# versmc/cmpt-eigenex

Measured on AMD Instinct MI355X. Metric: lanczos_krylov_iterations_per_second, higher is better.
Workload: dtype f64

## Files before the change

### cmpt-eigenex_amd/csrc/kernels.hip

```cpp
#include "kernels.hpp"

#include <algorithm>
#include <cstdlib>
#include <type_traits>

namespace eigenex {

namespace {

__device__ __forceinline__ double wave_sum(double x) {
#pragma unroll
  for (int off = 32; off > 0; off >>= 1) x += __shfl_down(x, off, 64);
  return x;
}

__device__ __forceinline__ double block_sum(double x, double* lds4) {
  x = wave_sum(x);
  const int lane = threadIdx.x & 63, wave = threadIdx.x >> 6;
  __syncthreads();
  if (lane == 0) lds4[wave] = x;
  __syncthreads();
  return (lds4[0] + lds4[1]) + (lds4[2] + lds4[3]);
}

// ... 243 lines not shown
  for (int i = threadIdx.x; i < (DUAL ? 8 : 4) * nacc; i += kBlock) lds[i] = 0.0;
  __syncthreads();
  double a = 0.0;
  if (fin.partials) {
    a = inline_fin_sum(fin, lds4);
    if (blockIdx.x == 0 && threadIdx.x == 0) {
      fin.out[0] = a;
      fin_alpha_apply(fin.ctrl, a, fin.series, fin.mode == kFinishAlphaFirst);
    }
  } else if (tt.uk) {
    a = *tt.a;
  }
  const double b = (tt.uk && tt.ukm1) ? *tt.b : 0.0;
  double* wave_acc = lds + wave * nacc;
  double* wave_acc2 = lds + (4 + wave) * nacc;
  for (int64_t tile = blockIdx.x; tile < ntiles; tile += gridDim.x) {
    const int64_t base = tile * kTileRows + 2 * threadIdx.x;
    if ((tile + 1) * kTileRows <= n)
      dots_tile<true, CPLX, RED4, DUAL>(src, tt, a, b, src2, cs, ncols, base, n, wave_acc, wave_acc2);
    else
      dots_tile<false, CPLX, RED4, DUAL>(src, tt, a, b, src2, cs, ncols, base, n, wave_acc, wave_acc2);
  }
  __syncthreads();
  for (int c = threadIdx.x; c < nacc; c += kBlock) {
    partials[(int64_t)c * pstride + blockIdx.x] = (lds[c] + lds[nacc + c]) + (lds[2 * nacc + c] + lds[3 * nacc + c]);
    if (DUAL) {
      const double* l2 = lds + 4 * nacc;
      partials2[(int64_t)c * pstride + blockIdx.x] = (l2[c] + l2[nacc + c]) + (l2[2 * nacc + c] + l2[3 * nacc + c]);
    }
  }
}

template <bool CPLX>
__device__ __forceinline__ void axmy8(double2 (&w)[4], const double* __restrict__ h, int ci, const double2 (&x)[4]) {
  if (!CPLX) {
    const double hr = h[ci];
#pragma unroll
    for (int i = 0; i < 4; ++i) {
      w[i].x = fma(-hr, x[i].x, w[i].x);
      w[i].y = fma(-hr, x[i].y, w[i].y);
    }
  } else {
    const double hr = h[2 * ci], hi = h[2 * ci + 1];
#pragma unroll
    for (int i = 0; i < 4; ++i) {
      w[i].x = fma(hi, x[i].y, fma(-hr, x[i].x, w[i].x));
      w[i].y = fma(-hi, x[i].x, fma(-hr, x[i].y, w[i].y));
    }
  }
}

template <bool FULL, bool CPLX>
__device__ __forceinline__ double update_tile(const double* src, double* dst,
                                              const ThreeTerm& tt, double a, double b, const ColumnSet& cs, int ncols,
                                              int ntail, const double* __restrict__ h, int64_t base, int64_t n) {
  double2 w[4], uk[4], ukm1[4];
  load_w0<FULL>(w, src, tt, a, b, base, n, &uk, &ukm1);
  const int nv = cs.count - ntail;
  auto from_memory = [&](int lo, int hi) {
    int ci = lo;
    for (; ci + 4 <= hi; ci += 4) {
      double2 x0[4], x1[4], x2[4], x3[4];
      load_col<FULL>(x0, column_ptr(cs, ci + 0), base, n);
      load_col<FULL>(x1, column_ptr(cs, ci + 1), base, n);
      load_col<FULL>(x2, column_ptr(cs, ci + 2), base, n);
      load_col<FULL>(x3, column_ptr(cs, ci + 3), base, n);
      axmy8<CPLX>(w, h, ci + 0, x0);
      axmy8<CPLX>(w, h, ci + 1, x1);
      axmy8<CPLX>(w, h, ci + 2, x2);
      axmy8<CPLX>(w, h, ci + 3, x3);
    }
    for (; ci < hi; ++ci) {
      double2 x0[4];
      load_col<FULL>(x0, column_ptr(cs, ci), base, n);
      axmy8<CPLX>(w, h, ci, x0);
    }
  };
  from_memory(0, nv);
  if (ntail == 2) axmy8<CPLX>(w, h, cs.count - 2, ukm1);
  if (ntail >= 1) axmy8<CPLX>(w, h, cs.count - 1, uk);
  from_memory(cs.count, ncols);
  double nrm = 0.0;
#pragma unroll
  for (int i = 0; i < 4; ++i) {
    const int64_t row = base + i * (2 * kBlock);
    if (FULL || row < n) {
      nt_st2(dst + row, w[i]);
      nrm = fma(w[i].x, w[i].x, nrm);
      nrm = fma(w[i].y, w[i].y, nrm);
    }
  }
  return nrm;
}

template <bool CPLX, bool RED>
__global__ __launch_bounds__(kBlock) void k_update(const double* src, double* dst, ThreeTerm tt, ColumnSet cs,
                                                   const double* __restrict__ h, int64_t n, int64_t ntiles,
                                                   double* __restrict__ partials, const Ctrl* __restrict__ ctrl, InlineReduce red) {
  extern __shared__ double h_lds[];
  __shared__ double lds4[4];
  if (ctrl->stopped) return;
  const int ncols = cs.count + cs.nq;
  const double a = tt.uk ? *tt.a : 0.0;
  const double b = (tt.uk && tt.ukm1) ? *tt.b : 0.0;
  const int ntail = tail_columns(tt, cs);
  if (RED) {
    for (int c = 0; c < red.ncoef; ++c) {
      const double* p = red.partials + (int64_t)c * red.pstride;
      double sc = 0.0;
      for (int bb = threadIdx.x; bb < red.nblocks; bb += kBlock) sc += p[bb];
      sc = block_sum(sc, lds4);
      if (threadIdx.x == 0) h_lds[c] = sc;
    }
    __syncthreads();
    if (blockIdx.x == 0)
      for (int c = threadIdx.x; c < red.ncoef; c += kBlock) red.out[c] = h_lds[c];
  }
  const double* hh = RED ? h_lds : h;
  double nrm = 0.0;
  for (int64_t tile = blockIdx.x; tile < ntiles; tile += gridDim.x) {
    const int64_t base = tile * kTileRows + 2 * threadIdx.x;
    if ((tile + 1) * kTileRows <= n)
      nrm += update_tile<true, CPLX>(src, dst, tt, a, b, cs, ncols, ntail, hh, base, n);
    else
      nrm += update_tile<false, CPLX>(src, dst, tt, a, b, cs, ncols, ntail, hh, base, n);
  }
  nrm = block_sum(nrm, lds4);
  if (threadIdx.x == 0) partials[blockIdx.x] = nrm;
}

__global__ __launch_bounds__(kBlock) void k_reduce(const double* __restrict__ partials, int pstride, int nblocks,
                                                   double* __restrict__ out, const Ctrl* __restrict__ ctrl) {
  __shared__ double lds4[4];
  if (ctrl->stopped) return;
  const double* p = partials + (int64_t)blockIdx.x * pstride;
  double s = 0.0;
  for (int b = threadIdx.x; b < nblocks; b += kBlock) s += p[b];
  s = block_sum(s, lds4);
  if (threadIdx.x == 0) out[blockIdx.x] = s;
}

__device__ __forceinline__ void lag_apply8(double2 (&u)[4], double2 (&w)[4], double cj, double fj, bool with_w, const double2 (&x)[4]) {
#pragma unroll
  for (int i = 0; i < 4; ++i) {
    u[i].x = fma(-cj, x[i].x, u[i].x);
    u[i].y = fma(-cj, x[i].y, u[i].y);
    if (with_w) {
      w[i].x = fma(-fj, x[i].x, w[i].x);
      w[i].y = fma(-fj, x[i].y, w[i].y);
    }
  }
}

template <bool FULL, bool CORRECT>
__device__ __forceinline__ double sweep_tile(const SweepStep& st, double scale, double a, double b, const double* cl, const double* fl,
                                             double* wave_acc, int64_t base, int64_t n) {
  const int lane = threadIdx.x & 63;
  const int k = st.k;
  const double* ukm1 = st.V + (int64_t)(k - 1) * st.ldv;
  double* ukcol = const_cast<double*>(st.V) + (int64_t)k * st.ldv;
  double2 w0[4], w[4], u[4], um[4];
#pragma unroll
  for (int i = 0; i < 4; ++i) {
    const int64_t row = base + i * (2 * kBlock);
    u[i] = w0[i] = w[i] = um[i] = make_double2(0.0, 0.0);
    if (FULL || row < n) {
      const double2 t = ld2(st.w + row);
      u[i] = make_double2(t.x * scale, t.y * scale);
      if (!CORRECT) {
        double2 s = ld2(st.v + row);
        s.x = fma(-a, u[i].x, s.x);
        s.y = fma(-a, u[i].y, s.y);
        if (k > 0) {
          um[i] = ld2(ukm1 + row);
          s.x = fma(-b, um[i].x, s.x);
          s.y = fma(-b, um[i].y, s.y);
        }
        w0[i] = w[i] = s;
      }
    }
  }
  const int nv = CORRECT ? k : (k > 0 ? k - 1 : 0);
  int ci = 0;
  for (; ci + 4 <= nv; ci += 4) {
    double2 x0[4], x1[4], x2[4], x3[4];
    load_col<FULL>(x0, st.V + (int64_t)(ci + 0) * st.ldv, base, n);
    load_col<FULL>(x1, st.V + (int64_t)(ci + 1) * st.ldv, base, n);
    load_col<FULL>(x2, st.V + (int64_t)(ci + 2) * st.ldv, base, n);
    load_col<FULL>(x3, st.V + (int64_t)(ci + 3) * st.ldv, base, n);
    if (!CORRECT) {
      double r0, r1, r2, r3, im;
      dotc8<false>(w0, x0, r0, im);
      dotc8<false>(w0, x1, r1, im);
      dotc8<false>(w0, x2, r2, im);
      dotc8<false>(w0, x3, r3, im);
      const double kr = wave_sum4(r0, r1, r2, r3, lane);
      if ((lane & 15) == 0) wave_acc[ci + (lane >> 4)] += kr;
    }
    lag_apply8(u, w, cl[ci + 0], CORRECT ? 0.0 : fl[ci + 0], !CORRECT, x0);
    lag_apply8(u, w, cl[ci + 1], CORRECT ? 0.0 : fl[ci + 1], !CORRECT, x1);
    lag_apply8(u, w, cl[ci + 2], CORRECT ? 0.0 : fl[ci + 2], !CORRECT, x2);
    lag_apply8(u, w, cl[ci + 3], CORRECT ? 0.0 : fl[ci + 3], !CORRECT, x3);
  }
  for (; ci < nv; ++ci) {
    double2 x0[4];
    load_col<FULL>(x0, st.V + (int64_t)ci * st.ldv, base, n);
    if (!CORRECT) {
      double r0, im;
      dotc8<false>(w0, x0, r0, im);
      r0 = wave_sum(r0);
      if (lane == 0) wave_acc[ci] += r0;
    }
    lag_apply8(u, w, cl[ci], CORRECT ? 0.0 : fl[ci], !CORRECT, x0);
  }
  double nrm = 0.0;
  if (!CORRECT) {
    double r0, r1 = 0.0, im;
    if (k > 0) {
      dotc8<false>(w0, um, r1, im);
      lag_apply8(u, w, cl[k - 1], fl[k - 1], true, um);
    }
    dotc8<false>(w0, u, r0, im);
    const double fk = fl[k];
#pragma unroll
    for (int i = 0; i < 4; ++i) {
      w[i].x = fma(-fk, u[i].x, w[i].x);
      w[i].y = fma(-fk, u[i].y, w[i].y);
    }
    r0 = wave_sum(r0);
    if (k > 0) r1 = wave_sum(r1);
    if (lane == 0) {
      wave_acc[k] += r0;
      if (k > 0) wave_acc[k - 1] += r1;
    }
  }
#pragma unroll
  for (int i = 0; i < 4; ++i) {
    const int64_t row = base + i * (2 * kBlock);
    if (FULL || row < n) {
      nt_st2(ukcol + row, u[i]);
      if (!CORRECT) {
        nt_st2(st.w + row, w[i]);
        nrm = fma(w[i].x, w[i].x, nrm);
        nrm = fma(w[i].y, w[i].y, nrm);
      }
    }
  }
  return nrm;
}

template <bool CORRECT>
__global__ __launch_bounds__(kBlock) void k_sweep(SweepStep st, InlineFin fin, int64_t n, int64_t ntiles, double* __restrict__ dpartials,
                                                  int pstride, double* __restrict__ npartials, const Ctrl* ctrl) {
  extern __shared__ double lds[];
  __shared__ double lds4[4];
  if (ctrl->stopped) return;
  const int k = st.k, nacc = k + 1;
  double* cl = lds + 4 * nacc;
  double* fl = cl + nacc;
  for (int i = threadIdx.x; i < 4 * nacc; i += kBlock) lds[i] = 0.0;
  for (int i = threadIdx.x; i < nacc; i += kBlock) cl[i] = i < k ? st.lag[kLagC + i] : 0.0;
  const double a = fin.partials ? inline_fin_sum(fin, lds4) : *st.a_raw;
  __syncthreads();
  const double da = lag_alpha_correction(k, st.beta, cl);
  if (!CORRECT) {
    for (int i = threadIdx.x; i < nacc; i += kBlock) {
      const double fi = lag_f_entry(i, k, st.alpha, st.beta, cl, a, da);
      fl[i] = fi;
      if (blockIdx.x == 0) st.lag[st.f_off + i] = fi;
    }
  }
  if (blockIdx.x == 0 && threadIdx.x == 0) {
    st.lag[0] = a;
    if (fin.partials) {
      fin.out[0] = a;
      fin_alpha_apply(fin.ctrl, a - da, fin.series, fin.mode == kFinishAlphaFirst);
    } else if (k > 0) {
      st.alpha[k] = a - da;
    }
  }
  __syncthreads();
  const double scale = *st.scale;
  const double b = k > 0 ? st.beta[k - 1] : 0.0;
  double* wave_acc = lds + (threadIdx.x >> 6) * nacc;
  double nrm = 0.0;
  for (int64_t tile = blockIdx.x; tile < ntiles; tile += gridDim.x) {
    const int64_t base = tile * kTileRows + 2 * threadIdx.x;
    if ((tile + 1) * kTileRows <= n)
      nrm += sweep_tile<true, CORRECT>(st, scale, a, b, cl, fl, wave_acc, base, n);
    else
      nrm += sweep_tile<false, CORRECT>(st, scale, a, b, cl, fl, wave_acc, base, n);
  }
  if (CORRECT) return;
  __syncthreads();
  for (int c = threadIdx.x; c < nacc; c += kBlock)
    dpartials[(int64_t)c * pstride + blockIdx.x] = (lds[c] + lds[nacc + c]) + (lds[2 * nacc + c] + lds[3 * nacc + c]);
  nrm = block_sum(nrm, lds4);
  if (threadIdx.x == 0) npartials[blockIdx.x] = nrm;
}

constexpr int kLagWaves = 16;
__global__ __launch_bounds__(64 * kLagWaves) void k_lag_terms(int k, const double* __restrict__ dpartials, int pstride, int nblocks,
                                                              const double* __restrict__ npartials, double* lag, int f_off, double threshold,
                                                              Ctrl* ctrl, Ctrl* repair) {
  __shared__ double lds4[4];
  __shared__ double wmax[kLagWaves];
  if (ctrl->stopped) {
    if (threadIdx.x == 0) repair->stopped = 1;
    return;
  }
  const int lane = threadIdx.x & 63, wave = threadIdx.x >> 6, nwaves = blockDim.x >> 6;
  if (wave < kBlock / 64) {
    double s = 0.0;
    for (int b = threadIdx.x; b < nblocks; b += kBlock) s += npartials[b];
    s = wave_sum(s);
    if (lane == 0) lds4[wave] = s;
  }
  __syncthreads();
  const double beta = sqrt((lds4[0] + lds4[1]) + (lds4[2] + lds4[3]));
  double m = 0.0;
  for (int c = wave; c <= k; c += nwaves) {
    const double* p = dpartials + (int64_t)c * pstride;
    double d = 0.0;
    for (int b = lane; b < nblocks; b += 64) d += p[b];
    d = wave_sum(d);
    if (lane == 0) {
      const double cc = lag_next_coefficient(d, lag[f_off + c], beta, threshold);
      lag[kLagC + c] = cc;
      m = fmax(m, fabs(cc));
    }
  }
  if (lane == 0) wmax[wave] = m;
  __syncthreads();
  double mx = 0.0;
  for (int w = 0; w < nwaves; ++w) mx = fmax(mx, wmax[w]);
  const bool armed = mx > kLagGuard;
  if (armed)
    for (int c = threadIdx.x; c <= k; c += blockDim.x) lag[kLagC + c] = 0.0;
  if (threadIdx.x == 0) {
    repair->stopped = armed ? 0 : 1;
    if (armed) ctrl->repairs++;
  }
}

__global__ void k_close_scalars(int k, const double* a_raw, double* alpha, const double* __restrict__ beta, double* lag, const Ctrl* __restrict__ ctrl) {
  if (ctrl->stopped) return;
  const double a = *a_raw;
  const double da = lag_alpha_correction(k, beta, lag + kLagC);
  lag[0] = a;
  if (k > 0) alpha[k] = a - da;
}

__device__ __forceinline__ void cheb_store(const ChebStep& ch, int64_t r, double a, double x) {
  const double tp = ch.first ? x : ch.t_prev[r];
  const double acc = ch.first ? 0.0 : ch.acc[r];
  double acc_new;
  const double t = cheb_row_nofma(a, tp, acc, ch, &acc_new);
  __builtin_nontemporal_store(t, &ch.t_next[r]);
  __builtin_nontemporal_store(acc_new, &ch.acc[r]);
}

template <bool FULL>
__device__ __forceinline__ void cheb_tile(const double* __restrict__ y, const ChebStep& ch, int64_t base, int64_t n) {
  double2 a[4], tp[4], ac[4];
#pragma unroll
  for (int i = 0; i < 4; ++i) {
    const int64_t row = base + i * (2 * kBlock);
    a[i] = tp[i] = ac[i] = make_double2(0.0, 0.0);
    if (FULL || row < n) {
      a[i] = nt_ld_d2(y + row);
      tp[i] = ld2(ch.t_prev + row);
      if (!ch.first) ac[i] = ld2(ch.acc + row);
    }
  }
#pragma unroll
  for (int i = 0; i < 4; ++i) {
    const int64_t row = base + i * (2 * kBlock);
    if (FULL || row < n) {
      double2 t, an;
      t.x = cheb_row_nofma(a[i].x, tp[i].x, ac[i].x, ch, &an.x);
      t.y = cheb_row_nofma(a[i].y, tp[i].y, ac[i].y, ch, &an.y);
      nt_st2(ch.t_next + row, t);
      nt_st2(ch.acc + row, an);
    }
  }
}

__global__ __launch_bounds__(kBlock) void k_cheb_combine(const double* __restrict__ y, ChebStep ch, int64_t n, int64_t ntiles,
                                                         const Ctrl* __restrict__ ctrl) {
  if (ctrl->stopped) return;
  for (int64_t tile = blockIdx.x; tile < ntiles; tile += gridDim.x) {
    const int64_t base = tile * kTileRows + 2 * threadIdx.x;
    if ((tile + 1) * kTileRows <= n)
      cheb_tile<true>(y, ch, base, n);
    else
      cheb_tile<false>(y, ch, base, n);
  }
}

__device__ __forceinline__ double moment_row_nofma(double a, double t_prev, const MomentStep& mo) {
#pragma clang fp contract(off)
  const double ca = mo.c * a;
  return mo.first ? ca : ca - t_prev;
}
__device__ __forceinline__ double moment_store(const MomentStep& mo, int64_t r, double a) {
  const double tp = mo.first ? 0.0 : mo.t_prev[r];
  const double t = moment_row_nofma(a, tp, mo);
  __builtin_nontemporal_store(t, &mo.t_next[r]);
  return t;
}

template <bool FULL>
__device__ __forceinline__ void moments_tile(const double* __restrict__ y, const MomentStep& mo, int64_t base, int64_t n, double* tt, double* tx) {
  double2 a[4], tp[4], x[4];
#pragma unroll
  for (int i = 0; i < 4; ++i) {
    const int64_t row = base + i * (2 * kBlock);
    a[i] = tp[i] = x[i] = make_double2(0.0, 0.0);
    if (FULL || row < n) {
      a[i] = nt_ld_d2(y + row);
      x[i] = ld2(mo.t_cur + row);
      if (!mo.first) tp[i] = ld2(mo.t_prev + row);
    }
  }
#pragma unroll
  for (int i = 0; i < 4; ++i) {
    const int64_t row = base + i * (2 * kBlock);
    if (FULL || row < n) {
      double2 t;
      t.x = moment_row_nofma(a[i].x, tp[i].x, mo);
      t.y = moment_row_nofma(a[i].y, tp[i].y, mo);
      nt_st2(mo.t_next + row, t);
      *tt = fma(t.x, t.x, *tt);
      *tt = fma(t.y, t.y, *tt);
      *tx = fma(t.x, x[i].x, *tx);
      *tx = fma(t.y, x[i].y, *tx);
    }
  }
}

__global__ __launch_bounds__(kBlock) void k_cheb_moments(const double* __restrict__ y, MomentStep mo, int64_t n, int64_t ntiles,
                                                         double* __restrict__ partials, const Ctrl* __restrict__ ctrl) {
  __shared__ double lds4[4];
  if (ctrl->stopped) return;
  double tt = 0.0, tx = 0.0;
// ... 1774 lines not shown
        a1[e].x = fma(-ci, v1.y, fma(cr, v1.x, a1[e].x));
        a1[e].y = fma(ci, v1.x, fma(cr, v1.y, a1[e].y));
      }
    }
#pragma unroll
    for (int e = 0; e < NE; ++e) {
      if (e < nev) {
        double* xp = X + (int64_t)e * ldx;
        if (in0) st2(xp + 2 * r0, a0[e]);
        if (in1) st2(xp + 2 * r1, a1[e]);
      }
    }
  }
}

__global__ __launch_bounds__(kBlock) void k_first_nonzero(const double* __restrict__ X, int64_t ldx, int64_t n, int es,
                                                          double* __restrict__ out) {
  __shared__ long long best[kBlock];
  const double* x = X + (int64_t)blockIdx.x * ldx;
  long long found = n;
  for (int64_t c0 = 0; c0 < n && found == n; c0 += kBlock * 16) {
    long long mine = n;
    for (int j = 0; j < 16; ++j) {
      const int64_t i = c0 + j * kBlock + threadIdx.x;
      if (i < n && i < mine) {
        const bool nz = es == 1 ? fabs(x[i]) > 0.0 : (fabs(x[2 * i]) > 0.0 || fabs(x[2 * i + 1]) > 0.0);
        if (nz) mine = i;
      }
    }
    best[threadIdx.x] = mine;
    __syncthreads();
    for (int s = kBlock / 2; s > 0; s >>= 1) {
      if (threadIdx.x < s && best[threadIdx.x + s] < best[threadIdx.x]) best[threadIdx.x] = best[threadIdx.x + s];
      __syncthreads();
    }
    found = best[0];
    __syncthreads();
  }
  if (threadIdx.x == 0) {
    out[3 * blockIdx.x] = (double)found;
    out[3 * blockIdx.x + 1] = found < n ? x[found * es] : 0.0;
    out[3 * blockIdx.x + 2] = (found < n && es == 2) ? x[found * es + 1] : 0.0;
  }
}

__global__ __launch_bounds__(kBlock) void k_scale_columns(double* __restrict__ X, int64_t ldx, int64_t n, int es,
                                                          const double* __restrict__ factors) {
  double* x = X + (int64_t)blockIdx.y * ldx;
  const double fr = factors[2 * blockIdx.y], fi = factors[2 * blockIdx.y + 1];
  for (int64_t i = (int64_t)blockIdx.x * kBlock + threadIdx.x; i < n; i += (int64_t)gridDim.x * kBlock) {
    if (es == 1) {
      x[i] *= fr;
    } else {
      const double a = x[2 * i], b = x[2 * i + 1];
      x[2 * i] = a * fr - b * fi;
      x[2 * i + 1] = a * fi + b * fr;
    }
  }
}

__global__ __launch_bounds__(kBlock) void k_ritz_combine(const double* __restrict__ X, int64_t ldx, int nc, int64_t n,
                                                         int es, double* __restrict__ out, int64_t ldo,
                                                         double* __restrict__ partials, int pstride) {
  __shared__ double lds4[4];
  for (int e = 0; e < nc; ++e) {
    const double* xa = X + (int64_t)(2 * e) * ldx;
    const double* xb = xa + ldx;
    double2* o = reinterpret_cast<double2*>(out) + (int64_t)e * ldo;
    double nrm = 0.0;
    for (int64_t i = (int64_t)blockIdx.x * kBlock + threadIdx.x; i < n; i += (int64_t)gridDim.x * kBlock) {
      double2 z;
      if (es == 1)
        z = make_double2(xa[i], xb[i]);
      else
        z = make_double2(xa[2 * i] - xb[2 * i + 1], xa[2 * i + 1] + xb[2 * i]);
      o[i] = z;
      nrm = fma(z.x, z.x, fma(z.y, z.y, nrm));
    }
    nrm = block_sum(nrm, lds4);
    if (threadIdx.x == 0) partials[(int64_t)e * pstride + blockIdx.x] = nrm;
  }
}

int g_num_cu = 256;

}

int grid_for_tiles(int64_t ntiles, int blocks_per_cu) {
  int64_t cap = (int64_t)g_num_cu * blocks_per_cu;
  int64_t g = ntiles < cap ? ntiles : cap;
  return g < 1 ? 1 : (int)g;
}

void set_num_cu(int n) { g_num_cu = n > 0 ? n : 256; }

void launch_dots(hipStream_t s, const double* src, ThreeTerm tt, ColumnSet cs, int64_t n, double* partials,
                 int pstride, int grid, const Ctrl* ctrl, bool cplx, const double* src2, double* partials2, const InlineFin* fin,
                 const InlineDecide* dec) {
  const int ncols = cs.count + cs.nq;
  if (ncols <= 0) return;
  const int64_t ntiles = (n + kTileRows - 1) / kTileRows;
  const size_t shmem = (size_t)(src2 ? 8 : 4) * ncols * (cplx ? 2 : 1) * sizeof(double);
  static const bool red4 = [] {
    const char* e = getenv("EIGENEX_DOTS_RED4");
    return e ? atoi(e) != 0 : true;
  }();
  const InlineFin nofin{nullptr, 0, 0, 0.0, nullptr, nullptr, nullptr};
  const InlineFin f = fin ? *fin : nofin;
  const InlineDecide nodec{nullptr, nullptr, 0, nullptr, 0, 0.0, nullptr, nullptr};
  const InlineDecide dd = dec ? *dec : nodec;
#define EIGENEX_LAUNCH_DOTS(C, R, D) \
  hipLaunchKernelGGL((k_dots<C, R, D>), dim3(grid), dim3(kBlock), shmem, s, src, tt, src2, cs, n, ntiles, partials, partials2, pstride, ctrl, f, dd)
  if (src2) {
    if (cplx)
      EIGENEX_LAUNCH_DOTS(true, true, true);
    else
      EIGENEX_LAUNCH_DOTS(false, true, true);
  } else if (cplx) {
    if (red4)
      EIGENEX_LAUNCH_DOTS(true, true, false);
    else
      EIGENEX_LAUNCH_DOTS(true, false, false);
  } else {
    if (red4)
      EIGENEX_LAUNCH_DOTS(false, true, false);
    else
      EIGENEX_LAUNCH_DOTS(false, false, false);
  }
#undef EIGENEX_LAUNCH_DOTS
}

void launch_update(hipStream_t s, const double* src, double* dst, ThreeTerm tt, ColumnSet cs, const double* h,
                   int64_t n, double* partials, int grid, const Ctrl* ctrl, bool cplx, const InlineReduce* red) {
  const int64_t ntiles = (n + kTileRows - 1) / kTileRows;
  const InlineReduce nored{nullptr, 0, 0, 0, nullptr};
  const InlineReduce r = red ? *red : nored;
  const size_t shmem = red ? sizeof(double) * (size_t)red->ncoef : 0;
  if (red && cplx)
    hipLaunchKernelGGL((k_update<true, true>), dim3(grid), dim3(kBlock), shmem, s, src, dst, tt, cs, h, n, ntiles, partials, ctrl, r);
  else if (red)
    hipLaunchKernelGGL((k_update<false, true>), dim3(grid), dim3(kBlock), shmem, s, src, dst, tt, cs, h, n, ntiles, partials, ctrl, r);
  else if (cplx)
    hipLaunchKernelGGL((k_update<true, false>), dim3(grid), dim3(kBlock), 0, s, src, dst, tt, cs, h, n, ntiles, partials, ctrl, r);
  else
    hipLaunchKernelGGL((k_update<false, false>), dim3(grid), dim3(kBlock), 0, s, src, dst, tt, cs, h, n, ntiles, partials, ctrl, r);
}

void launch_sweep(hipStream_t s, const SweepStep& st, const InlineFin* fin, int64_t n, double* dpartials, int pstride, double* npartials,
                  int grid, const Ctrl* ctrl) {
  const int64_t ntiles = (n + kTileRows - 1) / kTileRows;
  const size_t shmem = sizeof(double) * 6 * (size_t)(st.k + 1);
  const InlineFin nofin{nullptr, 0, 0, 0.0, nullptr, nullptr, nullptr};
  const InlineFin f = fin ? *fin : nofin;
  if (st.correct_only)
    hipLaunchKernelGGL(k_sweep<true>, dim3(grid), dim3(kBlock), shmem, s, st, f, n, ntiles, dpartials, pstride, npartials, ctrl);
  else
    hipLaunchKernelGGL(k_sweep<false>, dim3(grid), dim3(kBlock), shmem, s, st, f, n, ntiles, dpartials, pstride, npartials, ctrl);
}

void launch_lag_terms(hipStream_t s, int k, const double* dpartials, int pstride, int nblocks, const double* npartials, double* lag,
                      int f_off, double threshold, Ctrl* ctrl, Ctrl* repair) {
  const int waves = std::min(kLagWaves, std::max(kBlock / 64, k + 1));
  hipLaunchKernelGGL(k_lag_terms, dim3(1), dim3(64 * waves), 0, s, k, dpartials, pstride, nblocks, npartials, lag, f_off, threshold, ctrl, repair);
}

void launch_close_scalars(hipStream_t s, int k, const double* a_raw, double* alpha, const double* beta, double* lag, const Ctrl* ctrl) {
  hipLaunchKernelGGL(k_close_scalars, dim3(1), dim3(1), 0, s, k, a_raw, alpha, beta, lag, ctrl);
}

void launch_spmv_z(hipStream_t s, const int32_t* rowptr, const int32_t* col, const double* val, const double* x_ext,
                   const double* scale, double shift_re, double shift_im, double* y, double* u_out, int64_t n,
                   double* partials, int pstride, int grid, const Ctrl* ctrl, int spmv_flags, int pass) {
  const int64_t ntiles = (n + kSpmvRows - 1) / kSpmvRows;
  if (spmv_flags & kSpmvLongRows)
    hipLaunchKernelGGL(k_spmv_z<true>, dim3(grid), dim3(kBlock), 0, s, rowptr, col, reinterpret_cast<const double2*>(val),
                       reinterpret_cast<const double2*>(x_ext), scale, shift_re, shift_im, reinterpret_cast<double2*>(y),
                       reinterpret_cast<double2*>(u_out), n, ntiles, partials, pstride, spmv_flags, pass, ctrl);
  else
    hipLaunchKernelGGL(k_spmv_z<false>, dim3(grid), dim3(kBlock), 0, s, rowptr, col, reinterpret_cast<const double2*>(val),
                       reinterpret_cast<const double2*>(x_ext), scale, shift_re, shift_im, reinterpret_cast<double2*>(y),
                       reinterpret_cast<double2*>(u_out), n, ntiles, partials, pstride, spmv_flags, pass, ctrl);
}

void launch_shift_dot_z(hipStream_t s, double* y, const double* u, double shift_re, double shift_im, int64_t n,
                        double* partials, int pstride, int grid, const Ctrl* ctrl) {
  hipLaunchKernelGGL(k_shift_dot_z, dim3(grid), dim3(kBlock), 0, s, reinterpret_cast<double2*>(y),
                     reinterpret_cast<const double2*>(u), shift_re, shift_im, n, partials, pstride, ctrl);
}

void launch_reduce(hipStream_t s, const double* partials, int pstride, int nblocks, int ncols, double* out,
                   const Ctrl* ctrl) {
  if (ncols <= 0) return;
  hipLaunchKernelGGL(k_reduce, dim3(ncols), dim3(kBlock), 0, s, partials, pstride, nblocks, out, ctrl);
}

template <class OFF>
static void launch_spmv_t(hipStream_t s, const OFF* rowptr, const int32_t* col, const double* val, const double* x_ext,
                          const double* scale, double shift, double* y, double* u_out, int64_t n, double* partials, int grid,
                          const Ctrl* ctrl, int spmv_flags, int pass, const InlineFin* fin, const InlineArnoldiBegin* begin,
                          const int32_t* tile_list, int64_t list_len, const ChebStep* cheb, const MomentStep* mom) {
  const int64_t ntiles = tile_list ? list_len : (n + kSpmvRows - 1) / kSpmvRows;
  if (ntiles <= 0) return;
  const InlineFin nofin{nullptr, 0, 0, 0.0, nullptr, nullptr, nullptr};
  const InlineArnoldiBegin nobegin{nullptr, 0.0, 0, 0, nullptr, 0, 0, -1, nullptr, 0, nullptr, nullptr, nullptr, 0, nullptr, nullptr};
  const bool nt = (spmv_flags & 2) != 0;
  if (mom) {
#define EIGENEX_LAUNCH_SPMV_MOM(LONG, NTV)                                                                                                     \
  hipLaunchKernelGGL((k_spmv_moments<LONG, OFF, NTV>), dim3(grid), dim3(kBlock), 0, s, rowptr, col, val, x_ext, scale, shift, partials, n, ntiles, \
                     spmv_flags, ctrl, tile_list, *mom)
    if (spmv_flags & kSpmvLongRows) {
      if (nt) EIGENEX_LAUNCH_SPMV_MOM(true, true);
      else EIGENEX_LAUNCH_SPMV_MOM(true, false);
    } else {
      if (nt) EIGENEX_LAUNCH_SPMV_MOM(false, true);
      else EIGENEX_LAUNCH_SPMV_MOM(false, false);
    }
#undef EIGENEX_LAUNCH_SPMV_MOM
    return;
  }
  if (cheb) {
#define EIGENEX_LAUNCH_SPMV_CHEB(LONG, NTV)                                                                                                \
  hipLaunchKernelGGL((k_spmv_cheb<LONG, OFF, NTV>), dim3(grid), dim3(kBlock), 0, s, rowptr, col, val, x_ext, scale, shift, u_out, n, ntiles, \
                     spmv_flags, ctrl, tile_list, *cheb)
    if (spmv_flags & kSpmvLongRows) {
      if (nt) EIGENEX_LAUNCH_SPMV_CHEB(true, true);
      else EIGENEX_LAUNCH_SPMV_CHEB(true, false);
    } else {
      if (nt) EIGENEX_LAUNCH_SPMV_CHEB(false, true);
      else EIGENEX_LAUNCH_SPMV_CHEB(false, false);
    }
#undef EIGENEX_LAUNCH_SPMV_CHEB
    return;
  }
#define EIGENEX_LAUNCH_SPMV(LONG, NTV)                                                                                              \
  hipLaunchKernelGGL((k_spmv<LONG, OFF, NTV>), dim3(grid), dim3(kBlock), 0, s, rowptr, col, val, x_ext, scale, shift, y, u_out, n, \
                     ntiles, partials, spmv_flags, pass, ctrl, fin ? *fin : nofin, begin ? *begin : nobegin, tile_list)
  if (spmv_flags & kSpmvLongRows) {
    if (nt) EIGENEX_LAUNCH_SPMV(true, true);
    else EIGENEX_LAUNCH_SPMV(true, false);
  } else {
    if (nt) EIGENEX_LAUNCH_SPMV(false, true);
    else EIGENEX_LAUNCH_SPMV(false, false);
  }
#undef EIGENEX_LAUNCH_SPMV
}
void launch_spmv(hipStream_t s, const int32_t* rowptr, const int32_t* col, const double* val, const double* x_ext,
                 const double* scale, double shift, double* y, double* u_out, int64_t n, double* partials, int grid,
                 const Ctrl* ctrl, int spmv_flags, int pass, const InlineFin* fin, const InlineArnoldiBegin* begin,
                 const int32_t* tile_list, int64_t list_len, const ChebStep* cheb, const MomentStep* mom) {
  launch_spmv_t(s, rowptr, col, val, x_ext, scale, shift, y, u_out, n, partials, grid, ctrl, spmv_flags, pass, fin, begin, tile_list, list_len, cheb, mom);
}
void launch_spmv64(hipStream_t s, const int64_t* rowptr, const int32_t* col, const double* val, const double* x_ext,
                   const double* scale, double shift, double* y, double* u_out, int64_t n, double* partials, int grid,
                   const Ctrl* ctrl, int spmv_flags, int pass, const InlineFin* fin, const InlineArnoldiBegin* begin,
                   const int32_t* tile_list, int64_t list_len, const ChebStep* cheb, const MomentStep* mom) {
  launch_spmv_t(s, rowptr, col, val, x_ext, scale, shift, y, u_out, n, partials, grid, ctrl, spmv_flags, pass, fin, begin, tile_list, list_len, cheb, mom);
}
void launch_spmv_rows(hipStream_t s, const RowCodeView& op, const double* x_ext, const double* scale, double shift, double* y,
                      double* u_out, int64_t n, double* partials, int grid, const Ctrl* ctrl, int spmv_flags, int pass,
                      const InlineFin* fin, const InlineArnoldiBegin* begin, const int32_t* tile_list, int64_t list_len,
                      const ChebStep* cheb, const MomentStep* mom) {
  const int64_t ntiles = tile_list ? list_len : (n + kSpmvRows - 1) / kSpmvRows;
  if (ntiles <= 0) return;
  const InlineFin nofin{nullptr, 0, 0, 0.0, nullptr, nullptr, nullptr};
  const InlineArnoldiBegin nobegin{nullptr, 0.0, 0, 0, nullptr, 0, 0, -1, nullptr, 0, nullptr, nullptr, nullptr, 0, nullptr, nullptr};
  if (mom && op.rec_bytes == 8)
    hipLaunchKernelGGL(k_spmv_rows_moments<8>, dim3(grid), dim3(kBlock), 0, s, op, x_ext, scale, shift, partials, n, ntiles, spmv_flags, ctrl, tile_list, *mom);
  else if (mom)
    hipLaunchKernelGGL(k_spmv_rows_moments<16>, dim3(grid), dim3(kBlock), 0, s, op, x_ext, scale, shift, partials, n, ntiles, spmv_flags, ctrl, tile_list, *mom);
  else if (cheb && op.rec_bytes == 8)
    hipLaunchKernelGGL(k_spmv_rows_cheb<8>, dim3(grid), dim3(kBlock), 0, s, op, x_ext, scale, shift, u_out, n, ntiles, spmv_flags, ctrl, tile_list, *cheb);
  else if (cheb)
    hipLaunchKernelGGL(k_spmv_rows_cheb<16>, dim3(grid), dim3(kBlock), 0, s, op, x_ext, scale, shift, u_out, n, ntiles, spmv_flags, ctrl, tile_list, *cheb);
  else if (op.rec_bytes == 8)
    hipLaunchKernelGGL(k_spmv_rows<8>, dim3(grid), dim3(kBlock), 0, s, op, x_ext, scale, shift, y, u_out, n, ntiles, partials,
                       spmv_flags, pass, ctrl, fin ? *fin : nofin, begin ? *begin : nobegin, tile_list);
  else
    hipLaunchKernelGGL(k_spmv_rows<16>, dim3(grid), dim3(kBlock), 0, s, op, x_ext, scale, shift, y, u_out, n, ntiles, partials,
                       spmv_flags, pass, ctrl, fin ? *fin : nofin, begin ? *begin : nobegin, tile_list);
}

template <class OFF>
__global__ __launch_bounds__(kBlock) void k_encode_rows(const OFF* __restrict__ rowptr, const int32_t* __restrict__ col,
                                                        const double* __restrict__ val, int64_t n, int64_t nrec_rows, RowCodeSlots slots,
                                                        int nslots, RowCodePalette pal, int rec_bytes, uint8_t* __restrict__ rec,
                                                        unsigned int* bad) {
  for (int64_t r = (int64_t)blockIdx.x * kBlock + threadIdx.x; r < nrec_rows; r += (int64_t)gridDim.x * kBlock) {
    uint8_t b[kRowCodeMaxSlots];
    bool ok = true;
    if (r < n) {
      const OFF p = rowptr[r];
      ok = row_code_encode(r, col + p, val + p, (int64_t)(rowptr[r + 1] - p), slots.off, nslots, pal.bits, pal.n, b, rec_bytes);
    } else {
      for (int i = 0; i < rec_bytes; ++i) b[i] = (uint8_t)kRowCodeAbsent;
    }
    if (!ok) atomicAdd(bad, 1u);
    for (int i = 0; i < rec_bytes; ++i) rec[r * rec_bytes + i] = b[i];
  }
}
void launch_encode_rows(hipStream_t s, const int32_t* rowptr, const int64_t* rowptr64, const int32_t* col, const double* val, int64_t n,
                        int64_t nrec_rows, const RowCodeSlots& slots, int nslots, const RowCodePalette& pal, int rec_bytes, uint8_t* rec,
                        unsigned int* bad) {
  const int grid = (int)std::min<int64_t>((nrec_rows + kBlock - 1) / kBlock, 65536);
  if (grid <= 0) return;
  if (rowptr64)
    hipLaunchKernelGGL(k_encode_rows<int64_t>, dim3(grid), dim3(kBlock), 0, s, rowptr64, col, val, n, nrec_rows, slots, nslots, pal,
                       rec_bytes, rec, bad);
  else
    hipLaunchKernelGGL(k_encode_rows<int32_t>, dim3(grid), dim3(kBlock), 0, s, rowptr, col, val, n, nrec_rows, slots, nslots, pal,
                       rec_bytes, rec, bad);
// ... 348 lines not shown
```

### cmpt-eigenex_amd/csrc/kernels.hpp

```cpp
#pragma once
#include <hip/hip_runtime.h>
#include <stdint.h>

#include "lag_terms.hpp"
#include "row_codes.hpp"
#include "spin_measure.hpp"
#include "spin_rdm.hpp"
#include "spin_model.hpp"
#include "spin_momentum.hpp"
#include "spin_rows.hpp"
#include "spin_sector.hpp"
#include "spin_site.hpp"
#include "split_layout.hpp"
#include "spmv_index.hpp"

namespace eigenex {

struct Ctrl {
  int stopped;
  int nvec;
  int nalpha;
  int nbeta;
  int iterations;
  int calls_true;
  int keep_coupling;
  int repairs;
  double scale;
  double residue;
};

constexpr int kRowsPerThread = 8;
constexpr int kTileRows = kBlock * kRowsPerThread;

struct ColumnSet {
  const double* V;
  int64_t ldv;
  int first, stride, count;
  const double* Q;
  int64_t ldq;
  int nq;
};

struct ThreeTerm {
  const double* uk;
  const double* ukm1;
  const double* a;
  const double* b;
};

struct InlineFin {
  const double* partials;
  int nblocks;
  int mode;
  double threshold;
  double* series;
  Ctrl* ctrl;
  double* out;
};

struct InlineArnoldiBegin {
  Ctrl* ctrl;
  double threshold;
  int64_t n_global;
  int cap;
  double* H;
  int ldh, es;
  int tail_k;
  const double* tail_partials;
  int tail_nblocks;
  const Ctrl* pass2;
  double* h;
  const double* h2;
  int ncoef;
  const double* nrm2_first;
  double* nrm2_final;
};

struct InlineDecide {
  Ctrl* pass2;
  const double* after_partials;
  int after_n;
  const double* before_partials;
  int before_n;
  double eta2;
  double* nrm2_first;
  double* nrm2_before;
};

struct InlineReduce {
  const double* partials;
  int pstride, nblocks, ncoef;
  double* out;
};

struct ChebStep {
  const double* t_prev;
  double* t_next;
  double* acc;
  double c, mu0, mu;
  int first;
};

struct MomentStep {
  const double* t_prev;
  double* t_next;
  const double* t_cur;
  double c;
  int first;
  int pstride;
};

__host__ __device__ inline uint64_t random_sign_mix(uint64_t z) {
  z ^= z >> 30;
  z *= 0xBF58476D1CE4E5B9ull;
  z ^= z >> 27;
  z *= 0x94D049BB133111EBull;
  z ^= z >> 31;
  return z;
}
__host__ __device__ inline uint64_t random_sign_key(uint64_t seed, uint64_t stream) {
  const uint64_t G = 0x9E3779B97F4A7C15ull;
  return random_sign_mix((random_sign_mix(seed + G) ^ stream) + G);
}
__host__ __device__ inline bool random_sign_bit(uint64_t key, uint64_t row) { return (random_sign_mix((key ^ row) + 0x9E3779B97F4A7C15ull) >> 63) != 0; }

constexpr int kLagC = 8;
struct SweepStep {
  int k;
  const double* V;
  int64_t ldv;
  const double* v;
  double* w;
  const double* scale;
  const double* a_raw;
  double* alpha;
  const double* beta;
  double* lag;
  int f_off;
  int correct_only;
};
void launch_sweep(hipStream_t s, const SweepStep& st, const InlineFin* fin, int64_t n, double* dpartials, int pstride, double* npartials,
                  int grid, const Ctrl* ctrl);
void launch_lag_terms(hipStream_t s, int k, const double* dpartials, int pstride, int nblocks, const double* npartials, double* lag,
                      int f_off, double threshold, Ctrl* ctrl, Ctrl* repair);
void launch_close_scalars(hipStream_t s, int k, const double* a_raw, double* alpha, const double* beta, double* lag, const Ctrl* ctrl);

int grid_for_tiles(int64_t ntiles, int blocks_per_cu);
void set_num_cu(int n);

void launch_dots(hipStream_t s, const double* src, ThreeTerm tt, ColumnSet cs, int64_t n, double* partials,
                 int pstride, int grid, const Ctrl* ctrl, bool cplx, const double* src2 = nullptr, double* partials2 = nullptr,
                 const InlineFin* fin = nullptr, const InlineDecide* dec = nullptr);
void launch_form_h(hipStream_t s, Ctrl* ctrl, const double* fused, int ncoef, double* h, double* alpha, int first);
void launch_update(hipStream_t s, const double* src, double* dst, ThreeTerm tt, ColumnSet cs, const double* h,
                   int64_t n, double* partials, int grid, const Ctrl* ctrl, bool cplx, const InlineReduce* red = nullptr);
constexpr int kInlineReduceMaxCoef = 4096;
void launch_spmv_z(hipStream_t s, const int32_t* rowptr, const int32_t* col, const double* val, const double* x_ext,
                   const double* scale, double shift_re, double shift_im, double* y, double* u_out, int64_t n,
                   double* partials, int pstride, int grid, const Ctrl* ctrl, int spmv_flags = 0, int pass = 0);
void launch_shift_dot_z(hipStream_t s, double* y, const double* u, double shift_re, double shift_im, int64_t n,
                        double* partials, int pstride, int grid, const Ctrl* ctrl);
void launch_reduce(hipStream_t s, const double* partials, int pstride, int nblocks, int ncols, double* out,
                   const Ctrl* ctrl);
enum { kPassCarry = 1, kPassNotLast = 2, kPassSelfNorm = 4 };
enum { kSpmvLongRows = 4 };
void launch_spmv(hipStream_t s, const int32_t* rowptr, const int32_t* col, const double* val, const double* x_ext,
                 const double* scale, double shift, double* y, double* u_out, int64_t n, double* partials, int grid,
                 const Ctrl* ctrl, int spmv_flags = 0, int pass = 0, const InlineFin* fin = nullptr,
                 const InlineArnoldiBegin* begin = nullptr, const int32_t* tile_list = nullptr, int64_t list_len = 0,
                 const ChebStep* cheb = nullptr, const MomentStep* mom = nullptr);
void launch_spmv64(hipStream_t s, const int64_t* rowptr, const int32_t* col, const double* val, const double* x_ext,
                   const double* scale, double shift, double* y, double* u_out, int64_t n, double* partials, int grid,
                   const Ctrl* ctrl, int spmv_flags = 0, int pass = 0, const InlineFin* fin = nullptr,
                   const InlineArnoldiBegin* begin = nullptr, const int32_t* tile_list = nullptr, int64_t list_len = 0,
                   const ChebStep* cheb = nullptr, const MomentStep* mom = nullptr);
struct RowCodeView {
  const uint64_t* rec;
  const double* pal;
  int npal, rec_bytes;
  RowCodeSlots slots;
};
void launch_spmv_rows(hipStream_t s, const RowCodeView& op, const double* x_ext, const double* scale, double shift, double* y,
                      double* u_out, int64_t n, double* partials, int grid, const Ctrl* ctrl, int spmv_flags = 0, int pass = 0,
                      const InlineFin* fin = nullptr, const InlineArnoldiBegin* begin = nullptr, const int32_t* tile_list = nullptr,
                      int64_t list_len = 0, const ChebStep* cheb = nullptr, const MomentStep* mom = nullptr);
struct RowCodePalette {
  uint64_t bits[kRowCodeMaxValues];
  int n;
};
void launch_encode_rows(hipStream_t s, const int32_t* rowptr, const int64_t* rowptr64, const int32_t* col, const double* val, int64_t n,
                        int64_t nrec_rows, const RowCodeSlots& slots, int nslots, const RowCodePalette& pal, int rec_bytes, uint8_t* rec,
                        unsigned int* bad);
constexpr int kSortRows = 4096;
constexpr int kSortBlock = 1024;
constexpr int kSortCap = 8192;
constexpr int kSortBufDoubles = kSortCap + kSortCap / 32 + 8;
constexpr int kSortSliceElems = 32768;
struct SortedOperatorView {
  const int32_t* base;
  const uint32_t* cp;
  const double* val;
  const uint16_t* off;
  int nslices;
  int tile_rows;
  int slice_width;
  int64_t n_low, npad, nloc;
};
int sorted_grid(int64_t n, int tile_rows);
void launch_spmv_sorted(hipStream_t s, const SortedOperatorView& op, const double* x_ext, const double* scale, double shift, double* y,
                        double* u_out, int64_t n, double* partials, const Ctrl* ctrl, int pass = 0);
struct SplitOperatorView {
  const int32_t* wg_chunk;
  const int4* chunk;
  const uint32_t* cp;
  const double* val;
  int groups, tile_rows;
  int64_t n_low, npad, nloc;
  double* part;
  int64_t part_stride;
};
void launch_spmv_split_z(hipStream_t s, const SplitOperatorView& op, const double* x_ext, const double* scale, double shift_re,
                         double shift_im, double* y, double* u_out, int64_t n, double* partials, int pstride, const Ctrl* ctrl, int pass = 0);
int split_combine_grid(int64_t n);
bool prepare_spmv_split();
void launch_spmv_split(hipStream_t s, const SplitOperatorView& op, const double* x_ext, const double* scale, double shift, double* y,
                       double* u_out, int64_t n, double* partials, const Ctrl* ctrl, int pass = 0, const InlineArnoldiBegin* begin = nullptr);
struct BlockOperatorView {
  const double* bval;
  const int64_t* gent;
  const int64_t* gcol;
  const int32_t* cols;
  const int32_t* grow0;
  const int32_t* rowgrp;
};
void launch_block_spmv(hipStream_t s, const BlockOperatorView& op, const double* x_ext, const double* scale, double shift,
                       double* y, double* u_out, int64_t n, double* partials, int grid, const Ctrl* ctrl, int pass = 0);
void launch_block_spmv_z(hipStream_t s, const BlockOperatorView& op, const double* x_ext, const double* scale, double shift_re,
                         double shift_im, double* y, double* u_out, int64_t n, double* partials, int pstride, int grid,
                         const Ctrl* ctrl, int pass = 0);
void launch_spin_spmv(hipStream_t s, const SpinSectorView* op, const uint32_t* lo_rank, const uint32_t* hi_base, const double* x_ext,
                      const double* scale, double shift, double* y, double* u_out, int64_t n, double* partials, int grid, const Ctrl* ctrl,
                      int pass = 0);
void launch_spin_spmv_z(hipStream_t s, const SpinSectorView* op, const uint32_t* lo_rank, const uint32_t* hi_base, const double* x_ext,
                        const double* scale, double shift_re, double shift_im, double* y, double* u_out, int64_t n, double* partials,
                        int pstride, int grid, const Ctrl* ctrl, int pass = 0);
void launch_spin_measure(hipStream_t s, int es, const SpinMeasureChunk* chunk, const SpinSectorView* op, const uint32_t* lo_rank,
                         const uint32_t* hi_base, const double* x, int64_t n, double* partials, int pstride, int grid);
void launch_spin_measure_reduce(hipStream_t s, const double* partials, int pstride, int nblocks, int ndiag, int nflip, double* diag_out,
                                double* flip_out, double* norm_out);
void launch_spin_site_apply(hipStream_t s, int es, const SpinSiteTable* table, const SpinSectorView* dst_op, const uint32_t* src_lo,
                            const uint32_t* src_hi, const double* x, double* y, int64_t n, double* partials, int grid);
void launch_spin_rdm(hipStream_t s, int es, bool big, const SpinRdmTable* table, const SpinRdmItem* items, int n_items,
                     const SpinSectorView* op, const uint32_t* lo_rank, const uint32_t* hi_base, const double* x, double* partials);
void launch_spin_rdm_reduce(hipStream_t s, int es, const SpinRdmTable* table, int64_t total, const double* partials, double* out);
void launch_spin_momentum_spmv(hipStream_t s, int es, const SpinMomentumView* op, const uint32_t* reps, const uint32_t* bucket,
                               const double* x_ext, const double* scale, double shift_re, double shift_im, double* y, double* u_out, int64_t n,
                               double* partials, int pstride, int grid, const Ctrl* ctrl, int pass = 0);
void launch_spin_momentum_spmv(hipStream_t s, int es, const SpinMomentum64View* op, const uint64_t* reps, const uint32_t* bucket,
                               const double* x_ext, const double* scale, double shift_re, double shift_im, double* y, double* u_out, int64_t n,
                               double* partials, int pstride, int grid, const Ctrl* ctrl, int pass = 0);
void launch_spin_momentum_measure(hipStream_t s, int es, const SpinMomentumMeasureChunk* chunk, const uint32_t* reps, const double* x, int n_sites,
                                  int cell, int n_trans, int64_t n, double* partials, int pstride, int grid);
void launch_spin_momentum_measure(hipStream_t s, int es, const SpinMomentumMeasureChunk* chunk, const uint64_t* reps, const double* x, int n_sites,
                                  int cell, int n_trans, int64_t n, double* partials, int pstride, int grid);
void launch_spin_momentum_expand(hipStream_t s, int es, const SpinMomentumView* op, const SpinSectorView* dst_op, const uint32_t* reps,
                                 const uint32_t* bucket, const double* x, double* y, int64_t n, double* partials, int grid);
void launch_scale(hipStream_t s, const double* x, const double* scale_dev, double scale_host, double* out, int64_t n,
                  const Ctrl* ctrl);
void launch_shift_dot(hipStream_t s, double* y, const double* u, double shift, int64_t n, double* partials, int grid,
                      const Ctrl* ctrl);
void launch_cheb_combine(hipStream_t s, const double* y, const ChebStep& step, int64_t n, int grid, const Ctrl* ctrl);
void launch_cheb_moments(hipStream_t s, const double* y, const MomentStep& step, int64_t n, double* partials, int grid, const Ctrl* ctrl);
void launch_random_signs(hipStream_t s, double* out, int64_t n, int64_t row0, int es, uint64_t seed, uint64_t stream);
void launch_pack(hipStream_t s, const double* x, const int32_t* idx, int64_t count, int es, double* out,
                 const Ctrl* ctrl);
constexpr int kMaxLoopbackShards = 64;
struct PtrPack {
  double* p[kMaxLoopbackShards];
};
void launch_sum_shards(hipStream_t s, const PtrPack& bufs, int nshards, int n);

enum FinNormMode { kFinInit = 0, kFinLanczos = 1, kFinArnoldi = 2 };
enum FinAlphaMode { kFinishAlpha = 8, kFinishAlphaFirst = 9 };
void launch_reduce_fin(hipStream_t s, const double* partials, int pstride, int nblocks, int ncomp, double* out, Ctrl* ctrl,
                       int mode, double* series, double threshold);
void launch_fin_norm(hipStream_t s, Ctrl* ctrl, const double* nrm2, double threshold, int mode, double* beta);
void launch_fin_alpha(hipStream_t s, Ctrl* ctrl, const double* val, double* alpha, int first, int cap);
void launch_arnoldi_begin(hipStream_t s, Ctrl* ctrl, double threshold, int64_t n_global, int cap, double* H, int ldh,
                          int es);
void launch_arnoldi_end(hipStream_t s, Ctrl* ctrl, const double* h, double* H, int ldh, int es);
void launch_add_small(hipStream_t s, double* dst, const double* src, int n, const Ctrl* ctrl);
void launch_decide_second_pass(hipStream_t s, const Ctrl* ctrl, Ctrl* pass2, const double* nrm2_before, const double* nrm2_after, double eta2);
void launch_select_norm(hipStream_t s, const Ctrl* pass2, const double* nrm2_first, const double* nrm2_second, double* nrm2_final);
// ... 23 lines not shown
```

Before: 94.76.

## Park sweep tile outputs in LDS and release stores at wall-clock slot boundaries

```diff
diff --git a/cmpt-eigenex_amd/csrc/kernels.hip b/cmpt-eigenex_amd/csrc/kernels.hip
--- a/cmpt-eigenex_amd/csrc/kernels.hip
+++ b/cmpt-eigenex_amd/csrc/kernels.hip
@@ -419,9 +419,32 @@
   }
 }
 
-template <bool FULL, bool CORRECT>
+struct SweepPark {
+  double2* slots;
+  int64_t tile;
+  uint64_t slot;
+  int shift;
+};
+__device__ __forceinline__ void sweep_release(SweepPark& pk, double* ukcol, double* w, int64_t n) {
+  const int64_t pbase = pk.tile * kTileRows + 2 * threadIdx.x;
+#pragma unroll
+  for (int i = 0; i < 4; ++i) {
+    const int64_t row = pbase + i * (2 * kBlock);
+    if (row < n) {
+      nt_st2(ukcol + row, pk.slots[i * kBlock + threadIdx.x]);
+      nt_st2(w + row, pk.slots[(4 + i) * kBlock + threadIdx.x]);
+    }
+  }
+  pk.tile = -1;
+}
+__device__ __forceinline__ void sweep_release_at_boundary(SweepPark& pk, double* ukcol, double* w, int64_t n) {
+  if (pk.tile >= 0 && (wall_clock64() >> pk.shift) != pk.slot) sweep_release(pk, ukcol, w, n);
+}
+
+template <bool FULL, bool CORRECT, bool PARK = false>
 __device__ __forceinline__ double sweep_tile(const SweepStep& st, double scale, double a, double b, const double* cl, const double* fl,
-                                             double* wave_acc, int64_t base, int64_t n) {
+                                             double* wave_acc, int64_t base, int64_t n, SweepPark* pk = nullptr) {
+  static_assert(!(PARK && CORRECT), "the closing pass stores directly");
   const int lane = threadIdx.x & 63;
   const int k = st.k;
   const double* ukm1 = st.V + (int64_t)(k - 1) * st.ldv;
@@ -455,6 +478,7 @@
     load_col<FULL>(x1, st.V + (int64_t)(ci + 1) * st.ldv, base, n);
     load_col<FULL>(x2, st.V + (int64_t)(ci + 2) * st.ldv, base, n);
     load_col<FULL>(x3, st.V + (int64_t)(ci + 3) * st.ldv, base, n);
+    if (PARK) sweep_release_at_boundary(*pk, ukcol, st.w, n);
     if (!CORRECT) {
       double r0, r1, r2, r3, im;
       dotc8<false>(w0, x0, r0, im);
@@ -472,6 +496,7 @@
   for (; ci < nv; ++ci) {
     double2 x0[4];
     load_col<FULL>(x0, st.V + (int64_t)ci * st.ldv, base, n);
+    if (PARK) sweep_release_at_boundary(*pk, ukcol, st.w, n);
     if (!CORRECT) {
       double r0, im;
       dotc8<false>(w0, x0, r0, im);
@@ -500,6 +525,21 @@
       wave_acc[k] += r0;
       if (k > 0) wave_acc[k - 1] += r1;
     }
+  }
+  if (PARK) {
+    if (pk->tile >= 0) sweep_release(*pk, ukcol, st.w, n);
+#pragma unroll
+    for (int i = 0; i < 4; ++i) {
+      pk->slots[i * kBlock + threadIdx.x] = u[i];
+      pk->slots[(4 + i) * kBlock + threadIdx.x] = w[i];
+      const int64_t row = base + i * (2 * kBlock);
+      if (FULL || row < n) {
+        nrm = fma(w[i].x, w[i].x, nrm);
+        nrm = fma(w[i].y, w[i].y, nrm);
+      }
+    }
+    pk->slot = wall_clock64() >> pk->shift;
+    return nrm;
   }
 #pragma unroll
   for (int i = 0; i < 4; ++i) {
@@ -516,12 +556,14 @@
   return nrm;
 }
 
-template <bool CORRECT>
+template <bool CORRECT, bool PARK>
 __global__ __launch_bounds__(kBlock) void k_sweep(SweepStep st, InlineFin fin, int64_t n, int64_t ntiles, double* __restrict__ dpartials,
-                                                  int pstride, double* __restrict__ npartials, const Ctrl* ctrl) {
-  extern __shared__ double lds[];
+                                                  int pstride, double* __restrict__ npartials, const Ctrl* ctrl,
+                                                  int park_shift) {
+  extern __shared__ __align__(16) double lds_all[];
   __shared__ double lds4[4];
   if (ctrl->stopped) return;
+  double* lds = lds_all + (PARK ? kSweepParkBytes / (int)sizeof(double) : 0);
   const int k = st.k, nacc = k + 1;
   double* cl = lds + 4 * nacc;
   double* fl = cl + nacc;
@@ -551,13 +593,16 @@
   const double b = k > 0 ? st.beta[k - 1] : 0.0;
   double* wave_acc = lds + (threadIdx.x >> 6) * nacc;
   double nrm = 0.0;
+  SweepPark pk{reinterpret_cast<double2*>(lds_all), -1, 0, park_shift};
   for (int64_t tile = blockIdx.x; tile < ntiles; tile += gridDim.x) {
     const int64_t base = tile * kTileRows + 2 * threadIdx.x;
     if ((tile + 1) * kTileRows <= n)
-      nrm += sweep_tile<true, CORRECT>(st, scale, a, b, cl, fl, wave_acc, base, n);
+      nrm += sweep_tile<true, CORRECT, PARK>(st, scale, a, b, cl, fl, wave_acc, base, n, &pk);
     else
-      nrm += sweep_tile<false, CORRECT>(st, scale, a, b, cl, fl, wave_acc, base, n);
-  }
+      nrm += sweep_tile<false, CORRECT, PARK>(st, scale, a, b, cl, fl, wave_acc, base, n, &pk);
+    if (PARK) pk.tile = tile;
+  }
+  if (PARK && pk.tile >= 0) sweep_release(pk, const_cast<double*>(st.V) + (int64_t)k * st.ldv, st.w, n);
   if (CORRECT) return;
   __syncthreads();
   for (int c = threadIdx.x; c < nacc; c += kBlock)
@@ -2638,10 +2683,28 @@
   const size_t shmem = sizeof(double) * 6 * (size_t)(st.k + 1);
   const InlineFin nofin{nullptr, 0, 0, 0.0, nullptr, nullptr, nullptr};
   const InlineFin f = fin ? *fin : nofin;
-  if (st.correct_only)
-    hipLaunchKernelGGL(k_sweep<true>, dim3(grid), dim3(kBlock), shmem, s, st, f, n, ntiles, dpartials, pstride, npartials, ctrl);
-  else
-    hipLaunchKernelGGL(k_sweep<false>, dim3(grid), dim3(kBlock), shmem, s, st, f, n, ntiles, dpartials, pstride, npartials, ctrl);
+  static const bool direct = getenv("EIGENEX_SWEEP_DIRECT_STORES") != nullptr;
+  static const int shift = [] {
+    if (const char* e = getenv("EIGENEX_SWEEP_SLOT_SHIFT")) return std::min(62, std::max(0, atoi(e)));
+    int dev = 0, khz = 0;
+    if (hipGetDevice(&dev) != hipSuccess || hipDeviceGetAttribute(&khz, hipDeviceAttributeWallClockRate, dev) != hipSuccess || khz <= 0) khz = 100000;
+    int sh = 0;
+    while (sh < 40 && 1.5 * (double)((uint64_t)1 << sh) < kSweepSlotMicroseconds * 1e-3 * khz) ++sh;
+    return sh;
+  }();
+  if (st.correct_only) {
+    hipLaunchKernelGGL((k_sweep<true, false>), dim3(grid), dim3(kBlock), shmem, s, st, f, n, ntiles, dpartials, pstride, npartials, ctrl, 0);
+  } else if (direct || kSweepParkBytes + shmem + kSweepStaticLds > (size_t)kSweepLdsBudget) {
+    hipLaunchKernelGGL((k_sweep<false, false>), dim3(grid), dim3(kBlock), shmem, s, st, f, n, ntiles, dpartials, pstride, npartials, ctrl, 0);
+  } else {
+    static const bool big_lds = [] {
+      return hipFuncSetAttribute(reinterpret_cast<const void*>(&k_sweep<false, true>), hipFuncAttributeMaxDynamicSharedMemorySize,
+                                 kSweepLdsBudget - kSweepStaticLds) == hipSuccess;
+    }();
+    (void)big_lds;
+    hipLaunchKernelGGL((k_sweep<false, true>), dim3(grid), dim3(kBlock), kSweepParkBytes + shmem, s, st, f, n, ntiles, dpartials, pstride, npartials,
+                       ctrl, shift);
+  }
 }
 
 void launch_lag_terms(hipStream_t s, int k, const double* dpartials, int pstride, int nblocks, const double* npartials, double* lag,
diff --git a/cmpt-eigenex_amd/csrc/kernels.hpp b/cmpt-eigenex_amd/csrc/kernels.hpp
--- a/cmpt-eigenex_amd/csrc/kernels.hpp
+++ b/cmpt-eigenex_amd/csrc/kernels.hpp
@@ -139,6 +139,10 @@
   int f_off;
   int correct_only;
 };
+constexpr int kSweepParkBytes = 2 * kTileRows * (int)sizeof(double);
+constexpr int kSweepLdsBudget = 80 * 1024;
+constexpr int kSweepStaticLds = 4 * (int)sizeof(double);
+constexpr double kSweepSlotMicroseconds = 80.0;
 void launch_sweep(hipStream_t s, const SweepStep& st, const InlineFin* fin, int64_t n, double* dpartials, int pstride, double* npartials,
                   int grid, const Ctrl* ctrl);
 void launch_lag_terms(hipStream_t s, int k, const double* dpartials, int pstride, int nblocks, const double* npartials, double* lag,
```

New measurement: 97.07, median of 6. +2.4%, better.
